# SeanNaren/deepspeech.pytorch

Hardware: AMD Instinct MI355X
Metric: audio-seconds/sec (train step) (higher is better)
Workload: dtype bf16

## Files before the change

deepspeech/pytorch_amd/_lib.py:

```python
import ctypes as C
import os

HERE = os.path.dirname(os.path.abspath(__file__))
LIB_PATH = os.path.join(HERE, "libds2hip.so")

F32, BF16 = 0, 1
CELL_GRU, CELL_LSTM, CELL_RNN_TANH = 0, 1, 2

_vp, _i, _l, _f, _ll = C.c_void_p, C.c_int, C.c_long, C.c_float, C.c_longlong

SIGNATURES = {
    "ds2_version": (_i, []),
    "ds2_error_string": (C.c_char_p, [_i]),
    "ds2_gemm_nt": (_i, [_i, _vp, _vp, _vp, _vp, _i, _i, _i, _l, _l, _l, _i, _i, _l, _l, _l, _l, _i, _vp]),
    "ds2_gemm_nt_coresident": (_i, [_i, _vp, _vp, _vp, _vp, _i, _i, _i, _l, _l, _l, _i, _i, _l, _l, _l, _l, _i, _vp]),
    "ds2_gemm_nt_rows2": (_i, [_i, _vp, _vp, _i, _vp, _vp, _i, _i, _i, _l, _l, _l, _i, _i, _i, _vp]),
    "ds2_gemm8_nt": (_i, [_vp, _vp, _vp, _vp, _i, _i, _i, _l, _l, _l, _i, _vp]),
    "ds2_gemm8_tn_grouped": (_i, [_i, _vp, _vp, _vp, _vp, _vp, _vp, _vp, _vp, _vp, _vp, _vp, _i, _vp]),
    "ds2_gemm8_nt_rows": (_i, [_vp, _vp, _vp, _vp, _i, _i, _i, _l, _l, _l, _i, _vp, _i, _vp]),
    "ds2_gemm8_tn_grouped_rows": (_i, [_i, _vp, _vp, _vp, _vp, _vp, _vp, _vp, _vp, _vp, _vp, _vp, _i, _vp, _i, _vp]),
    "ds2_gemm8_wgrad_dx_rows": (_i, [_i, _vp, _vp, _vp, _vp, _vp, _vp, _vp, _vp, _vp, _vp, _vp, _i, _vp, _vp, _vp, _i, _i, _i, _l, _l, _l, _vp, _i, _vp]),
    "ds2_zero_pad_rows": (_i, [_i, _vp, _l, _i, _vp, _i, _i, _vp]),
    "ds2_gemm8_wgrad_dx": (_i, [_i, _vp, _vp, _vp, _vp, _vp, _vp, _vp, _vp, _vp, _vp, _vp, _i, _vp, _vp, _vp, _i, _i, _i, _l, _l, _l, _vp]),
    "ds2_norm_partials": (_i, [_l]),
    "ds2_bn_fwd": (_i, [_i, _i, _i, _vp, _vp, _l, _i, _l, _l, _i, _i, _i, _vp, _vp, _vp, _vp, _vp, _vp, _f, _f, _vp, _vp,
                        _vp, _vp, _vp, _vp]),
    "ds2_bn_bwd": (_i, [_i, _i, _vp, _vp, _vp, _l, _i, _l, _l, _l, _i, _i, _i, _vp, _vp, _vp, _vp, _vp, _vp, _vp, _vp, _vp]),
    "ds2_colsum": (_i, [_i, _vp, _l, _i, _l, _vp, _f, _vp, _vp]),
    "ds2_conv_rows": (_i, [_i, _vp, _vp]),
    "ds2_conv1_fwd": (_i, [_i, _vp, _vp, _vp, _vp, _vp, _i, _i, _i, _i, _vp]),
    "ds2_conv1_wgrad_ws_floats": (_l, [_i, _i, _i]),
    "ds2_conv1_wgrad": (_i, [_i, _vp, _vp, _vp, _i, _i, _i, _i, _vp, _vp]),
    "ds2_conv2_fwd_ws_bytes": (_l, [_i, _i, _i, _i]),
    "ds2_conv2_fwd": (_i, [_i, _vp, _vp, _vp, _vp, _vp, _i, _i, _i, _vp, _vp]),
    "ds2_conv2_dgrad": (_i, [_i, _vp, _vp, _vp, _vp, _i, _i, _i, _vp]),
    "ds2_conv2_wgrad_ws_floats": (_l, [_i, _i]),
    "ds2_conv2_wgrad": (_i, [_i, _vp, _vp, _vp, _i, _i, _i, _vp, _vp]),
    "ds2_rnn_gates": (_i, [_i]),
    "ds2_rnn_saved_planes": (_i, [_i]),
    "ds2_rnn_state_bytes": (_l, [_i, _i, _i]),
    "ds2_rnn_fwd": (_i, [_i, _i, _i, _i, _i, _i, _vp, _vp, _vp, _vp, _vp, _vp, _vp, _l, _vp, _vp, _vp, _vp, _vp]),
    "ds2_rnn_bwd": (_i, [_i, _i, _i, _i, _i, _i, _vp, _vp, _vp, _vp, _l, _vp, _vp, _vp, _vp, _vp, _vp, _vp, _vp, _vp]),
    "ds2_rnn_persist_plan": (_i, [_i, _i, _i, _i, _i, _i, C.c_uint, C.POINTER(_l)]),
    "ds2_rnn_persist_supported": (_i, [_i, _i, _i, _i, _i, C.c_uint]),
    "ds2_rnn_persist_shape_covered": (_i, [_i, _i, _i, _i, _i]),
    "ds2_rnn_persist_kind": (_i, [_i, _i, _i, _i, _i, C.c_uint]),
    "ds2_rnn_persist_ws_bytes": (_l, [_i, _i, _i, _i, _i, C.c_uint]),
    "ds2_rnn_persist_fwd": (_i, [_i, _i, _i, _i, _i, _i, _vp, _vp, _vp, _vp, _vp, _vp, _vp, _l, _vp, _vp, _vp, _vp, _vp, _vp, _vp]),
    "ds2_rnn_persist_bwd": (_i, [_i, _i, _i, _i, _i, _i, _vp, _vp, _vp, _vp, _l, _vp, _vp, _vp, _vp, _i, _vp, _vp, _vp, _vp]),
    "ds2_add2": (_i, [_i, _vp, _vp, _vp, _l, _vp]),
    "ds2_sum_slices": (_i, [_vp, _vp, _l, _i, _vp]),
    "ds2_transpose": (_i, [_i, _vp, _vp, _l, _i, _l, _l, _vp]),
    "ds2_split3_bf16": (_i, [_vp, _l, _l, _i, _i, _i, _vp, _l, _vp]),
    "ds2_cast_transpose_bf16": (_i, [_vp, _l, _i, _i, _i, _i, _i, _vp, _l, _vp, _l, _vp]),
    "ds2_small_weight_layouts": (_i, [_i, _vp, _vp, _vp, _i, _i, _vp, _vp, _vp, _vp, _vp, _vp, _vp]),
    "ds2_scale_by": (_i, [_vp, _vp, _l, _vp]),
    "ds2_copy_words": (_i, [_vp, _vp, _l, _vp]),
    "ds2_lookahead_fwd": (_i, [_i, _vp, _vp, _vp, _vp, _i, _i, _i, _i, _vp]),
    "ds2_lookahead_ws_floats": (_l, [_i, _i, _i, _i]),
    "ds2_lookahead_bwd": (_i, [_i, _vp, _vp, _vp, _vp, _vp, _vp, _i, _i, _i, _i, _vp, _vp]),
    "ds2_rnn_bias_grads": (_i, [_i, _i, _i, _i, _vp, _vp, _vp, _vp]),
# ... 69 lines not shown
```

deepspeech/pytorch_amd/csrc/ds2_norm.hip:

```cpp
#include "ds2_common.h"

namespace {

constexpr int NORM_RY = 8;
constexpr int NORM_CX = 32;

struct RowMap {
  int F, Tp;
  __device__ __forceinline__ void nt(long row, int& n, int& t) const {
    t = (int)(row % Tp);
    n = (int)(row / ((long)F * Tp));
  }
};

__device__ __forceinline__ float bn_affine(float x, float sc, float sh) { return __builtin_fmaf(x, sc, sh); }
__device__ __forceinline__ bool hardtanh_open(float y) { return y > 0.f && y < 20.f; }
__device__ __forceinline__ float bn_dx(float g, float xh, float sc, float k1, float k2) { return sc * __builtin_fmaf(-xh, k2, g - k1); }

struct RedMap {
  int cpb, rpx, chunk, rsub;
  bool ok;
  __device__ __forceinline__ RedMap(int chunks) {
    cpb = chunks < NORM_CX ? chunks : NORM_CX;
    rpx = NORM_CX / cpb;
// ... 28 lines not shown
                                                                float* __restrict__ psum, float* __restrict__ psq) {
  constexpr int V = Vec16<T>::N;
  __shared__ float red[NORM_RY][NORM_CX * V + 1];
  const RedMap m(C / V);
  float s[V], q[V];
#pragma unroll
  for (int i = 0; i < V; ++i) s[i] = q[i] = 0.f;
  if (m.ok) {
    for (long r = m.first_row(); r < R; r += m.row_step()) {
      float v[V];
      Vec16<T>::load(X + r * ld + (long)m.chunk * V, v);
#pragma unroll
      for (int i = 0; i < V; ++i) {
        s[i] += v[i];
        if (SQ) q[i] += v[i] * v[i];
      }
    }
  }
  float o[V];
  red_block<V>(red, m, s, o);
  if (threadIdx.y == 0 && m.rsub == 0 && m.ok) {
#pragma unroll
    for (int i = 0; i < V; ++i) psum[(long)blockIdx.y * C + (long)m.chunk * V + i] = o[i];
  }
  if (SQ) {
    red_block<V>(red, m, q, o);
    if (threadIdx.y == 0 && m.rsub == 0 && m.ok) {
#pragma unroll
      for (int i = 0; i < V; ++i) psq[(long)blockIdx.y * C + (long)m.chunk * V + i] = o[i];
    }
  }
}

constexpr int FIN_COLS = 32, FIN_SLICES = 8;
template <int NA>
__device__ __forceinline__ void finalize_sums(const float* const (&arr)[NA], int P, int C, int c, int py, double (&tot)[NA]) {
  __shared__ double sh[NA][FIN_SLICES][FIN_COLS];
  double acc[NA];
#pragma unroll
  for (int a = 0; a < NA; ++a) acc[a] = 0.0;
  if (c < C) {
#pragma unroll 8
    for (int p = py; p < P; p += FIN_SLICES) {
#pragma unroll
      for (int a = 0; a < NA; ++a) acc[a] += (double)arr[a][(long)p * C + c];
    }
  }
#pragma unroll
  for (int a = 0; a < NA; ++a) sh[a][py][threadIdx.x & (FIN_COLS - 1)] = acc[a];
  __syncthreads();
#pragma unroll
  for (int a = 0; a < NA; ++a) {
    double t = 0.0;
    if (py == 0) {
#pragma unroll
      for (int q = 0; q < FIN_SLICES; ++q) t += sh[a][q][threadIdx.x & (FIN_COLS - 1)];
    }
    tot[a] = t;
  }
}

__global__ void __launch_bounds__(256) k_colsum_finalize(const float* __restrict__ psum, int P, int C, float* __restrict__ out,
                                                          float scale) {
  const int c = blockIdx.x * FIN_COLS + (threadIdx.x & (FIN_COLS - 1)), py = threadIdx.x / FIN_COLS;
  const float* const arr[1] = {psum};
  double tot[1];
  finalize_sums<1>(arr, P, C, c, py, tot);
  if (py == 0 && c < C) out[c] = (float)(tot[0] * (double)scale);
}

__global__ void k_bn_finalize(const float* __restrict__ psum, const float* __restrict__ psq, int P, int C, double count,
                              const float* __restrict__ gamma, const float* __restrict__ beta, float eps,
                              float momentum, float* __restrict__ running_mean, float* __restrict__ running_var,
                              long long* __restrict__ num_batches_tracked, float* __restrict__ mean_out,
                              float* __restrict__ rstd_out, float* __restrict__ scale_out, float* __restrict__ shift_out) {
  const int c = blockIdx.x * FIN_COLS + (threadIdx.x & (FIN_COLS - 1)), py = threadIdx.x / FIN_COLS;
  if (blockIdx.x == 0 && threadIdx.x == 0 && num_batches_tracked) *num_batches_tracked += 1;
  const float* const arr[2] = {psum, psq};
  double tot[2];
  finalize_sums<2>(arr, P, C, c, py, tot);
  if (py != 0 || c >= C) return;
  const double s = tot[0], q = tot[1];
  double mean = s / count;
  double var = q / count - mean * mean;
  if (var < 0.0) var = 0.0;
  double rstd = 1.0 / sqrt(var + (double)eps);
  mean_out[c] = (float)mean;
  rstd_out[c] = (float)rstd;
  float sc = (float)((double)gamma[c] * rstd);
  scale_out[c] = sc;
  shift_out[c] = (float)((double)beta[c] - mean * (double)gamma[c] * rstd);
  if (running_mean) {
    double unb = count > 1.0 ? var * (count / (count - 1.0)) : var;
    running_mean[c] = (float)((1.0 - (double)momentum) * (double)running_mean[c] + (double)momentum * mean);
    running_var[c] = (float)((1.0 - (double)momentum) * (double)running_var[c] + (double)momentum * unb);
  }
}

__global__ void k_bn_eval_coeffs(int C, const float* __restrict__ gamma, const float* __restrict__ beta,
                                 const float* __restrict__ running_mean, const float* __restrict__ running_var, float eps,
                                 float* __restrict__ scale_out, float* __restrict__ shift_out) {
  int c = blockIdx.x * blockDim.x + threadIdx.x;
  if (c >= C) return;
  double rstd = 1.0 / sqrt((double)running_var[c] + (double)eps);
  scale_out[c] = (float)((double)gamma[c] * rstd);
  shift_out[c] = (float)((double)beta[c] - (double)running_mean[c] * (double)gamma[c] * rstd);
}

template <typename T, bool CONV, bool SEQ_OUT, bool CENTRED = false>
__global__ void __launch_bounds__(256) k_bn_apply(const T* __restrict__ X, T* __restrict__ Y, long R, int C, long ldx,
                                                   long ldy, const float* __restrict__ scale,
                                                   const float* __restrict__ shift, const float* __restrict__ mean,
                                                   const float* __restrict__ beta, RowMap rm,
                                                   const int* __restrict__ lens, int N) {
  constexpr int V = Vec16<T>::N;
  const int chunks = C / V;
  const long total = R * chunks;
  for (long e = (long)blockIdx.x * blockDim.x + threadIdx.x; e < total; e += (long)gridDim.x * blockDim.x) {
    long r = e / chunks;
    int c0 = (int)(e % chunks) * V;
    float v[V];
    bool live = true;
    int n = 0, t = 0;
    if (CONV) {
      rm.nt(r, n, t);
// ... 225 lines not shown
  else
    hipLaunchKernelGGL((k_colstats<T, false>), grd, blk, 0, st, (const T*)X, R, C, ld, psum, psq);
  *P_out = grd.y;
  DS2_CHECK_LAUNCH();
  return 0;
}

inline int apply_grid(long total) {
  long g = (total + 255) / 256;
  if (g > 256 * 8) g = 256 * 8;
  if (g < 1) g = 1;
  return (int)g;
}

}

extern "C" {

int ds2_norm_partials(long R) { return norm_grid_y(R); }

int ds2_colsum(int dtype, const void* X, long R, int C, long ld, float* out, float scale, float* ws, ds2_stream_t st_) {
  hipStream_t st = (hipStream_t)st_;
  int P = 0, rc;
  if (dtype == DS2_F32)
    rc = colstats_impl<float>(X, R, C, ld, ws, nullptr, &P, st);
  else
    rc = colstats_impl<bf16_t>(X, R, C, ld, ws, nullptr, &P, st);
  if (rc) return rc;
  hipLaunchKernelGGL(k_colsum_finalize, dim3(ds2_cdiv(C, FIN_COLS)), dim3(256), 0, st, ws, P, C, out, scale);
  DS2_CHECK_LAUNCH();
  return 0;
}

int ds2_bn_fwd(int dtype, int mode, int training, const void* X, void* Y, long R, int C, long ldx, long ldy, int F, int Tp,
               int N, const int* lens, const float* gamma, const float* beta, float* running_mean, float* running_var,
               long long* num_batches_tracked, float eps, float momentum, float* save_mean, float* save_rstd,
               float* save_scale, float* save_shift, float* ws, ds2_stream_t st_) {
  hipStream_t st = (hipStream_t)st_;
  DS2_REQUIRE(dtype == DS2_F32 || dtype == DS2_BF16, DS2_ERR_DTYPE);
  DS2_REQUIRE(mode >= 0 && mode <= 2, DS2_ERR_ARG);
  DS2_REQUIRE(mode == 0 || R < (1L << 31), DS2_ERR_ARG);
  int rc, P = 0;
  if (training) {
    float* psum = ws;
    float* psq = ws + (long)norm_grid_y(R) * C;
    rc = dtype == DS2_F32 ? colstats_impl<float>(X, R, C, ldx, psum, psq, &P, st)
                          : colstats_impl<bf16_t>(X, R, C, ldx, psum, psq, &P, st);
    if (rc) return rc;
    hipLaunchKernelGGL(k_bn_finalize, dim3(ds2_cdiv(C, FIN_COLS)), dim3(256), 0, st, psum, psq, P, C, (double)R, gamma, beta,
                       eps, momentum, running_mean, running_var, num_batches_tracked, save_mean, save_rstd, save_scale,
                       save_shift);
  } else {
    hipLaunchKernelGGL(k_bn_eval_coeffs, dim3(ds2_cdiv(C, 128)), dim3(128), 0, st, C, gamma, beta, running_mean,
                       running_var, eps, save_scale, save_shift);
  }
  DS2_CHECK_LAUNCH();
  RowMap rm{F, Tp};
  const int V = dtype == DS2_F32 ? 4 : 8;
  DS2_REQUIRE(C % V == 0 && ldx % V == 0 && ldy % V == 0, DS2_ERR_ALIGN);
  dim3 g(apply_grid(R * (C / V))), b(256);
#define LAUNCH_APPLY(TT)                                                                                              \
  if (mode == 0 && training && R == 1)                                                                                \
    hipLaunchKernelGGL((k_bn_apply<TT, false, false, true>), g, b, 0, st, (const TT*)X, (TT*)Y, R, C, ldx, ldy,        \
                       save_scale, save_shift, save_mean, beta, rm, lens, N);                                         \
  else if (mode == 0)                                                                                                 \
    hipLaunchKernelGGL((k_bn_apply<TT, false, false>), g, b, 0, st, (const TT*)X, (TT*)Y, R, C, ldx, ldy, save_scale,  \
                       save_shift, save_mean, beta, rm, lens, N);                                                     \
  else if (mode == 1)                                                                                                 \
    hipLaunchKernelGGL((k_bn_apply<TT, true, false>), g, b, 0, st, (const TT*)X, (TT*)Y, R, C, ldx, ldy, save_scale,   \
                       save_shift, save_mean, beta, rm, lens, N);                                                     \
  else                                                                                                                \
    hipLaunchKernelGGL((k_bn_apply<TT, true, true>), g, b, 0, st, (const TT*)X, (TT*)Y, R, C, ldx, ldy, save_scale,    \
                       save_shift, save_mean, beta, rm, lens, N);
  if (dtype == DS2_F32) {
    LAUNCH_APPLY(float)
  } else {
    LAUNCH_APPLY(bf16_t)
  }
#undef LAUNCH_APPLY
  DS2_CHECK_LAUNCH();
  return 0;
}

int ds2_bn_bwd(int dtype, int mode, const void* G, const void* X, void* DX, long R, int C, long ldg, long ldx, long lddx,
               int F, int Tp, int N, const int* lens, const float* save_mean, const float* save_rstd,
               const float* save_scale, const float* save_shift, float* dgamma, float* dbeta, float* ws, ds2_stream_t st_) {
  hipStream_t st = (hipStream_t)st_;
  DS2_REQUIRE(dtype == DS2_F32 || dtype == DS2_BF16, DS2_ERR_DTYPE);
  DS2_REQUIRE(mode >= 0 && mode <= 2, DS2_ERR_ARG);
  DS2_REQUIRE(mode == 0 || R < (1L << 31), DS2_ERR_ARG);
  const int V = dtype == DS2_F32 ? 4 : 8;
  DS2_REQUIRE(C % V == 0 && ldx % V == 0 && ldg % V == 0 && lddx % V == 0, DS2_ERR_ALIGN);
  RowMap rm{F, Tp};
  const int P = norm_grid_y(R, ds2_cdiv(C / V, NORM_CX));
  float* ps = ws;
  float* pq = ws + (long)P * C;
  float* c1 = pq + (long)P * C;
  float* c2 = c1 + C;
  dim3 blk(NORM_CX, NORM_RY), grd(ds2_cdiv(C / V, NORM_CX), P);
#define LAUNCH_RED(TT, CV, SI)                                                                                          \
  hipLaunchKernelGGL((k_bn_bwd_reduce<TT, CV, SI>), grd, blk, 0, st, (const TT*)G, (const TT*)X, R, C, ldg, ldx,          \
                     save_scale, save_shift, save_mean, save_rstd, rm, lens, N, ps, pq)
  const int acb = ds2_cdiv(C / V, NORM_CX), arpx = NORM_CX / (C / V < NORM_CX ? C / V : NORM_CX);
  long agy = ds2_cdiv(R, (long)NORM_RY * arpx * 2);
  if (agy > 2048 / acb) agy = 2048 / acb;
  if (agy < 1) agy = 1;
  const dim3 agrd(acb, (unsigned)agy);
#ifdef DS2_BN_APPLY_GRIDSTRIDE
#define LAUNCH_APP(TT, CV, SI)                                                                                          \
  hipLaunchKernelGGL((k_bn_bwd_apply<TT, CV, SI>), dim3(apply_grid(R*(C / V))), dim3(256), 0, st, (const TT*)G,           \
                     (const TT*)X, (TT*)DX, R, C, ldg, ldx, lddx, save_scale, save_shift, save_mean, save_rstd, c1, c2, \
                     rm, lens, N)
// ... 30 lines not shown
```

deepspeech/pytorch_amd/model.py:

```python
import math
from typing import List

import numpy as np
import torch
import torch.nn as nn

from . import ops
from ._lib import Ds2HipError

try:
    import pytorch_lightning as pl
    _Base = pl.LightningModule
except Exception:
    pl = None

    class _Base(nn.Module):

        def save_hyperparameters(self, *a, **k):
            import inspect
            frame = inspect.currentframe().f_back
            try:
                names = [n for n in inspect.signature(type(self).__init__).parameters if n != "self"]
                self._hparams = {n: frame.f_locals[n] for n in names if n in frame.f_locals}
            finally:
# ... 159 lines not shown
    def clear(self):
        self._store.clear()


def _wgrad_splitk(M, N, K):
    tiles = ((M + 127) // 128) * ((N + 127) // 128)
    if tiles >= 128:
        return 1
    return max(1, min(8, 768 // max(tiles, 1), K // (64 * 32)))


def _pad_gate_rows(w, G, H, Hp):
    if Hp == H:
        return w
    out = w.new_zeros((G, Hp) + tuple(w.shape[1:]))
    out[:, :H] = w.reshape((G, H) + tuple(w.shape[1:]))
    return out.reshape((G * Hp,) + tuple(w.shape[1:]))


def _pad_cols(w, Cp):
    if w.shape[-1] == Cp:
        return w
    out = w.new_zeros(tuple(w.shape[:-1]) + (Cp,))
    out[..., :w.shape[-1]] = w
    return out


def _unpad_gate_rows(g, G, H, Hp):
    if Hp == H:
        return g
    return g.reshape((G, Hp) + tuple(g.shape[1:]))[:, :H].reshape((G * H,) + tuple(g.shape[1:])).contiguous()


def _bn_seq_fwd(bn, w, b, X, Xh, R, Ct, Cp, training):
    if Ct == Cp:
        return ops.bn_fwd(X, 0, training, w.detach(), b.detach(), bn.running_mean, bn.running_var, bn.num_batches_tracked, R, Ct,
                          X.stride(0), Xh, Xh.stride(0), eps=bn.eps, momentum=bn.momentum)
    g, be = w.new_ones(Cp), w.new_zeros(Cp)
    rm, rv = w.new_zeros(Cp), w.new_ones(Cp)
    g[:Ct], be[:Ct], rm[:Ct], rv[:Ct] = w.detach(), b.detach(), bn.running_mean, bn.running_var
    sv = ops.bn_fwd(X, 0, training, g, be, rm, rv, bn.num_batches_tracked, R, Cp, X.stride(0), Xh, Xh.stride(0), eps=bn.eps,
                    momentum=bn.momentum)
    if training:
        bn.running_mean.copy_(rm[:Ct])
        bn.running_var.copy_(rv[:Ct])
    return sv


def _bn_seq_bwd(G, X, DX, sv, R, Ct, Cp):
    dg, db = ops.bn_bwd(G, X, DX, 0, sv, R, Cp, G.stride(0), X.stride(0), DX.stride(0))
    return (dg, db) if Ct == Cp else (dg[:Ct].contiguous(), db[:Ct].contiguous())


def _perm_cols_to_internal(w):
    g, rin = w.shape
    out = w.new_zeros((g, _round64(rin)))
    out[:, :rin] = w.reshape(g, 32, rin // 32).permute(0, 2, 1).reshape(g, rin)
    return out


def _perm_cols_to_reference(w, rin=RNN_INPUT):
    g = w.shape[0]
    return w[:, :rin].reshape(g, rin // 32, 32).permute(0, 2, 1).reshape(g, rin)


class _ConvStackFn(torch.autograd.Function):

# ... 73 lines not shown
    R = Tp * N
    layer = mod.rnns[li]
    kind, Ht, D = layer.kind, layer.hidden_size, layer.num_directions
    H = mod._Hp
    G = ops.GATES[kind]
    first = li == 0
    I = mod._rnn_ld if first else H
    has_bn = layer.batch_norm is not None
    bn_w, bn_b = (lparams[0], lparams[1]) if has_bn else (None, None)
    wts = lparams[2 if has_bn else 0:]
    wih = [wts[4 * d + 0] for d in range(D)]
    whh = [wts[4 * d + 1] for d in range(D)]
    bih = [wts[4 * d + 2] for d in range(D)]
    bhh = [wts[4 * d + 3] for d in range(D)]

    def build_ih():
        w = torch.cat([_pad_gate_rows(p.detach(), G, Ht, H) for p in wih], 0)
        w = _perm_cols_to_internal(w) if first else _pad_cols(w, H)
        out = ops.empty_padded(w.shape[0], w.shape[1], dtype, w.device)
        out.copy_(w)
        return out
    Wih = c.get(("wih", li, dtype), wih, build_ih)
    Whh = c.get(("whh", li, dtype), whh, lambda: torch.stack(
        [_pad_gate_rows(_pad_cols(p.detach(), H), G, Ht, H) for p in whh], 0).to(dtype).contiguous())
    if H == Ht:
        Bih, Bhh = mod._bias_views(li)
    else:
        Bih = c.get(("bih", li), bih, lambda: torch.cat([_pad_gate_rows(p.detach(), G, Ht, H) for p in bih], 0))
        Bhh = c.get(("bhh", li), bhh, lambda: torch.stack([_pad_gate_rows(p.detach(), G, Ht, H) for p in bhh], 0))
    sv, Xh = None, X
    if has_bn:
        bn = layer.batch_norm.module
        Xh = ops.empty_padded(R, I, X.dtype, X.device)
        sv = _bn_seq_fwd(bn, bn_w, bn_b, X, Xh, R, layer.input_size, I, training)
    if ops.split3_ok(dtype, R, D * G * H, I):
        Wih3 = c.get(("wih3", li), wih, lambda: ops.split3(Wih, 1))
        GI = ops.gemm_nt(ops.split3(Xh, 0), Wih3, bias=Bih, out_dtype=torch.float32, rows=rows)
    else:
        GI = ops.gemm_nt(Xh, Wih, bias=Bih, rows=rows)
    if H != Ht:
        h0 = _pad_cols(h0, H) if h0 is not None else None
        c0 = _pad_cols(c0, H) if c0 is not None else None
    hext, Sv, hn, cn = ops.rnn_fwd(kind, GI, Whh, Bhh, lens_dev, D, N, H, Tp, h0=h0, c0=c0)
    if H != Ht:
        hn = hn[..., :Ht].contiguous()
        cn = cn[..., :Ht].contiguous() if cn is not None else None
    del GI
    if D == 2:
        out = ops.add2(hext[0, 1:Tp + 1].reshape(R, H), hext[1, 1:Tp + 1].reshape(R, H))
    else:
        out = hext[0, 1:Tp + 1].reshape(R, H)
    return out, hn, cn, [X, Xh if has_bn else None, hext, Sv], (kind, H, D, G, I, has_bn, sv, Ht, layer.input_size)


def _rnn_layer_backward(mod, li, meta, saved, lparams, dout, lens_dev, N, Tp, dtype, main, side, rows=None, state=None):
    kind, H, D, G, I, has_bn, sv, Ht, It = meta
    if state is not None:
        h0, c0, want = state
        h0p = _pad_cols(h0, H) if (h0 is not None and H != Ht) else h0
        c0p = _pad_cols(c0, H) if (c0 is not None and H != Ht) else c0
        state = (h0p, c0p, bool(want))
    dX, grads, rg = _rnn_layer_backward_impl(mod, li, meta, saved, lparams, dout, lens_dev, N, Tp, dtype, main, side, rows, state)
    if state is None:
        return dX, grads, None
    main.wait_stream(side)
    GH, po = G * H, (2 if has_bn else 0)
    if h0p is not None:
        n4 = (N + 3) // 4 * 4
        ar = torch.arange(N, device=lens_dev.device)
        for d in range(D):
            t_first = torch.zeros_like(ar) if d == 0 else (lens_dev.long().clamp(1, Tp) - 1)
            src = rg.dGH[d].reshape(Tp * N, GH) if (kind == "gru" and rg.dGH is not None) else rg.dGI[:, d * GH:(d + 1) * GH]
            g_first = src.index_select(0, t_first * N + ar).float()
            A = torch.zeros((GH, n4), dtype=torch.float32, device=g_first.device)
            A[:, :N] = g_first.t()
            B = torch.zeros((H, n4), dtype=torch.float32, device=g_first.device)
            B[:, :N] = h0p[d].t()
            corr = ops.gemm_nt(A, B, out_dtype=torch.float32)
            grads[po + 4 * d + 1] = grads[po + 4 * d + 1] + _unpad_gate_rows(corr, G, Ht, H)[:, :Ht]
    dstate = None
    if want:
        dstate = (rg.dh0[..., :Ht].contiguous(), rg.dc0[..., :Ht].contiguous() if rg.dc0 is not None else None)
# ... 512 lines not shown
            nn.BatchNorm2d(32),
            nn.Hardtanh(0, 20, inplace=True)
        ))
        rnn_input_size = int(math.floor((self.spect_cfg.sample_rate * self.spect_cfg.window_size) / 2) + 1)
        rnn_input_size = int(math.floor(rnn_input_size + 2 * 20 - 41) / 2 + 1)
        rnn_input_size = int(math.floor(rnn_input_size + 2 * 10 - 21) / 2 + 1)
        rnn_input_size *= 32
        self._F0 = int(math.floor((self.spect_cfg.sample_rate * self.spect_cfg.window_size) / 2) + 1)
        self._F1, self._F2 = ops.conv_rows(self._F0)
        self._rnn_in, self._rnn_ld = 32 * self._F2, _round64(32 * self._F2)
        if rnn_input_size != self._rnn_in or self._F2 < 1:
            raise ValueError("unsupported spectrogram geometry: %d frequency bins" % self._F0)
        self.rnns = nn.Sequential(
            BatchRNN(rnn_input_size, H, kind, bidirectional=self.bidirectional, batch_norm=False),
            *(BatchRNN(H, H, kind, bidirectional=self.bidirectional) for _ in range(L - 1))
        )
        self.lookahead = nn.Sequential(
            Lookahead(H, context=model_cfg.lookahead_context),
            nn.Hardtanh(0, 20, inplace=True)
        ) if not self.bidirectional else None
        fully_connected = nn.Sequential(nn.BatchNorm1d(H), nn.Linear(H, num_classes, bias=False))
        self.fc = nn.Sequential(SequenceWise(fully_connected))
        self.blank_index = self.labels.index('_')
        from .decoder import GreedyDecoder
        self.inference_softmax = InferenceBatchSoftmax()
        self.criterion = CTCLossHip(blank=self.blank_index)
        self.evaluation_decoder = GreedyDecoder(self.labels, blank_index=self.blank_index)
        self.wer, self.cer = _reference_metrics(self.evaluation_decoder)
        self._cache = _WeightCache()
        self._flat_bias = {}
        self._side_streams = {}
        self._prep_done = None
        self._frame_rows = None
        self._weights_dirty = False
        self._kind = kind

    def _prep_rnn_weights(self, dtype, need_backward):
        c = self._cache
        if self._Hp != self.rnns[0].hidden_size:
            return
        for li, layer in enumerate(self.rnns):
            p, D, first = layer.rnn, layer.num_directions, li == 0
            sufs = [""] + (["_reverse"] if D == 2 else [])
            wih = [getattr(p, "weight_ih_l0" + s_) for s_ in sufs]
            whh = [getattr(p, "weight_hh_l0" + s_) for s_ in sufs]
            bih = [getattr(p, "bias_ih_l0" + s_) for s_ in sufs]
            bhh = [getattr(p, "bias_hh_l0" + s_) for s_ in sufs]

            if dtype == torch.bfloat16:
                keys = [("wih", li, dtype), ("whh", li, dtype)]
                if need_backward:
                    keys += [("wihT", li, dtype), ("whhT", li, dtype)]
                if not all(c.valid(k, wih if k[0].startswith("wih") else whh) for k in keys):
                    GH, H = whh[0].shape
                    I = wih[0].shape[1]
                    Io = self._rnn_ld if first else I
                    perm = (32, self._F2) if first else None
                    dev = wih[0].device
                    Wih = ops.empty_padded(D * GH, Io, dtype, dev)
                    Whh = torch.empty((D, GH, H), dtype=dtype, device=dev)
                    WihT = torch.empty((Io, D * GH), dtype=dtype, device=dev) if need_backward else None
                    WhhT = torch.empty((D, H, GH), dtype=dtype, device=dev) if need_backward else None
                    with torch.no_grad():
                        for d in range(D):
                            ops.cast_transpose_bf16(wih[d].detach(), Wih[d * GH:], Wih.stride(0),
                                                    WihT[:, d * GH:] if need_backward else None, D * GH, perm=perm, cout=Io)
# ... 225 lines not shown
```

deepspeech/pytorch_amd/ops.py:

```python
import ctypes as C

import numpy as np
import torch

from . import _lib
from ._lib import F32, BF16, call, query

CELLS = {"gru": _lib.CELL_GRU, "lstm": _lib.CELL_LSTM, "rnn": _lib.CELL_RNN_TANH}
GATES = {"gru": 3, "lstm": 4, "rnn": 1}
SAVED_PLANES = {"gru": 4, "lstm": 5, "rnn": 0}


def dt(t):
    d = t if isinstance(t, torch.dtype) else t.dtype
    if d == torch.float32:
        return F32
    if d == torch.bfloat16:
        return BF16
    raise TypeError("ds2hip supports float32 and bfloat16 activations, got %s" % d)


def vecw(dtype):
    return 4 if dtype == torch.float32 else 8

# ... 260 lines not shown
    return out


def cast_transpose_bf16(src, dst=None, ldd=0, dstT=None, lddT=0, perm=None, cout=None):
    R, Cc = src.shape
    pc, pf = perm if perm is not None else (0, 0)
    call("ds2_cast_transpose_bf16", PF(src), src.stride(0), R, Cc, pc, pf, Cc if cout is None else cout,
         P(dst) if dst is not None else None, ldd, P(dstT) if dstT is not None else None, lddT, S())


def small_weight_layouts(w1, w2, wfc, dtype):
    dev, Cc, H = w1.device, wfc.shape[0], wfc.shape[1]
    w1k = torch.empty((451, 32), dtype=torch.float32, device=dev)
    w2t = torch.empty((21, 11, 32, 32), dtype=dtype, device=dev)
    w2d0 = torch.empty((11, 11, 32, 32), dtype=dtype, device=dev)
    w2d1 = torch.empty((10, 11, 32, 32), dtype=dtype, device=dev)
    wp = torch.empty((32, H), dtype=dtype, device=dev)
    wpT = torch.empty((H, 32), dtype=dtype, device=dev)
    call("ds2_small_weight_layouts", dt(dtype), PF(w1), PF(w2), PF(wfc), Cc, H, P(w1k), P(w2t), P(w2d0), P(w2d1), P(wp), P(wpT), S())
    return w1k, w2t, [w2d0, w2d1], wp, wpT


def scale_by_(x, s):
    call("ds2_scale_by", P(x), PF(s.reshape(1)), x.numel(), S())
    return x


def add2(a, b):
    out = torch.empty_like(a)
    call("ds2_add2", dt(a), P(a), P(b), P(out), a.numel(), S())
    return out


class BnSaved:
    __slots__ = ("mean", "rstd", "scale", "shift")

    def __init__(self, Cc, device):
        buf = torch.empty((4, Cc), dtype=torch.float32, device=device)
        self.mean, self.rstd, self.scale, self.shift = buf[0], buf[1], buf[2], buf[3]


def bn_fwd(X, mode, training, gamma, beta, rmean, rvar, nbt, R, Cc, ldx, Y, ldy, F=0, Tp=0, N=0, lens=None, eps=1e-5,
           momentum=0.1):
    sv = BnSaved(Cc, X.device)
    ws = torch.empty(2 * query("ds2_norm_partials", R) * Cc, dtype=torch.float32, device=X.device)
    call("ds2_bn_fwd", dt(X), mode, 1 if training else 0, P(X), P(Y), R, Cc, ldx, ldy, F, Tp, N, P(lens), PF(gamma), PF(beta),
         PF(rmean), PF(rvar), P(nbt) if training else C.c_void_p(0), float(eps), float(momentum), P(sv.mean), P(sv.rstd),
         P(sv.scale), P(sv.shift), P(ws), S())
    return sv


def bn_bwd(G, X, DX, mode, sv, R, Cc, ldg, ldx, lddx, F=0, Tp=0, N=0, lens=None):
    dgamma = torch.empty(Cc, dtype=torch.float32, device=X.device)
    dbeta = torch.empty(Cc, dtype=torch.float32, device=X.device)
    ws = torch.empty((2 * query("ds2_norm_partials", R) + 2) * Cc, dtype=torch.float32, device=X.device)
    call("ds2_bn_bwd", dt(X), mode, P(G), P(X), P(DX), R, Cc, ldg, ldx, lddx, F, Tp, N, P(lens), P(sv.mean), P(sv.rstd),
         P(sv.scale), P(sv.shift), P(dgamma), P(dbeta), P(ws), S())
    return dgamma, dbeta


def conv_rows(F0):
    F1 = (F0 + 2 * 20 - 41) // 2 + 1
    return F1, (F1 + 2 * 10 - 21) // 2 + 1


def conv1_fwd(x, w1k, b1, lens, Tp, dtype):
    N, _, F0, T = x.shape
    y1 = torch.empty((N, conv_rows(F0)[0], Tp, 32), dtype=dtype, device=x.device)
    call("ds2_conv1_fwd", dt(dtype), PF(x), PF(w1k), PF(b1), P(lens), P(y1), N, F0, T, Tp, S())
    return y1


def conv1_wgrad(x, dy1, Tp):
    N, _, F0, T = x.shape
    dw = torch.empty((451, 32), dtype=torch.float32, device=x.device)
    ws = torch.empty(query("ds2_conv1_wgrad_ws_floats", N, F0, Tp), dtype=torch.float32, device=x.device)
    call("ds2_conv1_wgrad", dt(dy1), P(x), P(dy1), P(dw), N, F0, T, Tp, P(ws), S())
    return dw


def conv2_fwd(a1, w2t, b2, lens, F0=161):
# ... 220 lines not shown
def use_persistent(kind, dtype, D, N, H):
    if not PERSIST_ENABLED:
        return False
    ok = bool(query("ds2_rnn_persist_supported", dt(dtype), CELLS[kind], D, N, H, int(_OPTS["variant"])))
    if ok:
        return True
    import os
    import warnings
    covered = bool(query("ds2_rnn_persist_shape_covered", dt(dtype), CELLS[kind], D, N, H))
    if covered:
        dev = torch.cuda.current_device()
        cus = torch.cuda.get_device_properties(dev).multi_processor_count
        if os.environ.get("DS2_ALLOW_LAUNCH_PER_STEP", "0") in ("", "0"):
            raise _lib.Ds2HipError("ds2hip: device %d exposes %d compute units (< 256): the persistent recurrent kernels need one "
                                   "workgroup per CU, all co-resident.  Set DS2_ALLOW_LAUNCH_PER_STEP=1 to run the launch-per-time-step "
                                   "kernels instead (several times slower)." % (dev, cus))
        if dev not in _WARNED_CUS:
            _WARNED_CUS.add(dev)
            warnings.warn("ds2hip: device %d exposes %d compute units (< 256): the persistent recurrent kernels are disabled, the "
                          "recurrent sweeps use one launch per time step" % (dev, cus))
    elif H >= PERSIST_CLIFF_MIN_H:
        key = (kind, str(dtype), D, N, H)
        if key not in _WARNED_SHAPES:
            _WARNED_SHAPES.add(key)
            widths = [w for w in range(16, 2049, 16) if query("ds2_rnn_persist_shape_covered", dt(dtype), CELLS[kind], D, N, w)]
            warnings.warn("ds2hip: no persistent recurrent kernel is instantiated for %s %s hidden=%d, %d direction(s), batch %d: the "
                          "sweeps run one launch per time step (5-8x slower per step).  For this cell, type, direction count and batch "
                          "persistent kernels exist with hidden in {%s}; the model class zero-pads other hidden sizes up to the nearest "
                          "instantiated width when that is at most 1.5x as wide (DS2_PAD_HIDDEN)."
                          % (str(dtype).replace("torch.", ""), kind, H, D, N, ", ".join(map(str, widths))))
    return False


def rnn_fwd(kind, GI, Whh, bhh, lens, D, N, H, Tp, h0=None, c0=None, save=True):
    dev, dtype = GI.device, GI.dtype
    hext = torch.empty((D, Tp + 2, N, H), dtype=dtype, device=dev)
    persistent = use_persistent(kind, dtype, D, N, H)
    if not persistent:
        hext[:, 0].zero_()
        hext[:, Tp + 1].zero_()
    ns = SAVED_PLANES[kind]
    Sv = torch.empty((D, Tp, N, max(ns, 1) * H) if ns else (1,), dtype=dtype, device=dev)
    hn = torch.empty((D, N, H), dtype=torch.float32, device=dev)
    cn = torch.empty((D, N, H), dtype=torch.float32, device=dev) if kind == "lstm" else None
    if persistent:
        ws = torch.empty(query("ds2_rnn_persist_ws_bytes", dt(dtype), CELLS[kind], D, N, H, int(_OPTS["variant"])), dtype=torch.uint8, device=dev)
        global LAST_PERSIST_WS
        LAST_PERSIST_WS = ws
        po = _persist_opts()
        with _sweep_timer("rnn_fwd_persistent", Tp):
            call("ds2_rnn_persist_fwd", dt(dtype), CELLS[kind], D, N, H, Tp, P(lens), P(GI), P(Whh), PF(bhh), PF(h0), PF(c0),
                 P(hext[:, 1]), (Tp + 2) * N * H, P(Sv), P(hn), P(cn), P(ws), P(_persist_err(dev)), C.byref(po), S())
        return hext, Sv, hn, cn
    state = torch.empty(query("ds2_rnn_state_bytes", D, N, H), dtype=torch.uint8, device=dev)
    with _sweep_timer("rnn_fwd", Tp):
        call("ds2_rnn_fwd", dt(dtype), CELLS[kind], D, N, H, Tp, P(lens), P(GI), P(Whh), PF(bhh), PF(h0), PF(c0),
             P(hext[:, 1]), (Tp + 2) * N * H, P(Sv), P(hn), P(cn), P(state), S())
    return hext, Sv, hn, cn


class RnnGrads:
    __slots__ = ("dGI", "dGH", "dQ", "bacc", "dh0", "dc0")

    def __init__(self, dGI, dGH=None, dQ=None, bacc=None):
        self.dGI, self.dGH, self.dQ, self.bacc = dGI, dGH, dQ, bacc
        self.dh0 = self.dc0 = None

    def tensors(self):
        return [t for t in (self.dGI, self.dGH, self.dQ, self.bacc) if t is not None]
# ... 340 lines not shown
```

include/ds2hip.h:

```cpp
#ifndef DS2HIP_H
#define DS2HIP_H

#include <stdint.h>

#ifdef __cplusplus
extern "C" {
#endif

typedef void* ds2_stream_t;

enum { DS2_F32 = 0, DS2_BF16 = 1 };
enum { DS2_CELL_GRU = 0, DS2_CELL_LSTM = 1, DS2_CELL_RNN_TANH = 2 };
enum {
  DS2_OK = 0,
  DS2_ERR_DTYPE = 1001,
  DS2_ERR_ARG = 1002,
  DS2_ERR_ALIGN = 1003
};

int ds2_version(void);
const char* ds2_error_string(int code);

int ds2_gemm_nt(int dtype, const void* A, const void* B, void* C, const float* bias, int M, int N, int K, long lda, long ldb,
                long ldc, int out_f32, int batch, long strideA, long strideB, long strideC, long strideBias, int splitk,
// ... 1 lines not shown

int ds2_gemm_nt_rows2(int dtype, const void* A, const void* A2, int m_split, const void* B, void* C, int M, int N, int K, long lda,
                      long ldb, long ldc, int out_f32, int splitk, int coresident, ds2_stream_t stream);
int ds2_gemm_nt_coresident(int dtype, const void* A, const void* B, void* C, const float* bias, int M, int N, int K, long lda,
                           long ldb, long ldc, int out_f32, int batch, long strideA, long strideB, long strideC, long strideBias,
                           int splitk, ds2_stream_t stream);

int ds2_gemm8_nt(const void* A, const void* B, void* C, const float* bias, int M, int N, int K, long lda, long ldb, long ldc, int out_f32,
                 ds2_stream_t stream);
int ds2_gemm8_tn_grouped(int n_problems, const void* const* At, const void* const* At2, const int* m_split, const void* const* Bt, void* const* C,
                         const int* M, const int* N, const long* lda, const long* lda2, const long* ldb, const long* ldc, int K, ds2_stream_t stream);

int ds2_gemm8_wgrad_dx(int n_tn, const void* const* At, const void* const* At2, const int* m_split, const void* const* Bt, void* const* C,
                       const int* M, const int* N, const long* lda, const long* lda2, const long* ldb, const long* ldc, int K_tn,
                       const void* A_nt, const void* B_nt, void* C_nt, int M_nt, int N_nt, int K_nt, long lda_nt, long ldb_nt, long ldc_nt,
                       ds2_stream_t stream);

int ds2_gemm8_nt_rows(const void* A, const void* B, void* C, const float* bias, int n_phys, int N, int K, long lda, long ldb, long ldc,
                      int out_f32, const int* rows, int n_rows, ds2_stream_t stream);
int ds2_gemm8_tn_grouped_rows(int n_problems, const void* const* At, const void* const* At2, const int* m_split, const void* const* Bt,
                              void* const* C, const int* M, const int* N, const long* lda, const long* lda2, const long* ldb, const long* ldc,
                              int n_phys, const int* rows, int n_rows, ds2_stream_t stream);
int ds2_gemm8_wgrad_dx_rows(int n_tn, const void* const* At, const void* const* At2, const int* m_split, const void* const* Bt, void* const* C,
                            const int* M, const int* N, const long* lda, const long* lda2, const long* ldb, const long* ldc, int K_tn,
                            const void* A_nt, const void* B_nt, void* C_nt, int M_nt, int N_nt, int K_nt, long lda_nt, long ldb_nt, long ldc_nt,
                            const int* rows, int n_rows, ds2_stream_t stream);
int ds2_zero_pad_rows(int dtype, void* X, long ld, int cols, const int* lens, int Tp, int N, ds2_stream_t stream);

int ds2_norm_partials(long R);
int ds2_bn_fwd(int dtype, int mode, int training, const void* X, void* Y, long R, int C, long ldx, long ldy, int F, int Tp,
               int N, const int* lens, const float* gamma, const float* beta, float* running_mean, float* running_var,
               long long* num_batches_tracked, float eps, float momentum, float* save_mean, float* save_rstd,
               float* save_scale, float* save_shift, float* ws, ds2_stream_t stream);
int ds2_bn_bwd(int dtype, int mode, const void* G, const void* X, void* DX, long R, int C, long ldg, long ldx, long lddx,
               int F, int Tp, int N, const int* lens, const float* save_mean, const float* save_rstd,
               const float* save_scale, const float* save_shift, float* dgamma, float* dbeta, float* ws,
               ds2_stream_t stream);
int ds2_colsum(int dtype, const void* X, long R, int C, long ld, float* out, float scale, float* ws, ds2_stream_t stream);

int ds2_conv_rows(int F0, int* F1, int* F2);
int ds2_conv1_fwd(int dtype, const float* x, const float* w1k, const float* b1, const int* lens, void* y1, int N, int F0, int T,
                  int Tp, ds2_stream_t stream);
long ds2_conv1_wgrad_ws_floats(int N, int F0, int Tp);
int ds2_conv1_wgrad(int dtype, const float* x, const void* dy1, float* dw1k, int N, int F0, int T, int Tp, float* ws,
                    ds2_stream_t stream);
long ds2_conv2_fwd_ws_bytes(int dtype, int N, int F0, int Tp);
int ds2_conv2_fwd(int dtype, const void* a1, const void* w2t, const float* b2, const int* lens, void* y2, int N, int F0, int Tp,
                  void* ws, ds2_stream_t stream);
int ds2_conv2_dgrad(int dtype, const void* dy2, const void* w2d_even, const void* w2d_odd, void* da1, int N, int F0, int Tp,
                    ds2_stream_t stream);
long ds2_conv2_wgrad_ws_floats(int N, int Tp);
int ds2_conv2_wgrad(int dtype, const void* dy2, const void* a1, float* dw2t, int N, int F0, int Tp, float* ws, ds2_stream_t stream);

int ds2_rnn_gates(int cell);
int ds2_rnn_saved_planes(int cell);
long ds2_rnn_state_bytes(int D, int N, int H);
int ds2_rnn_fwd(int dtype, int cell, int D, int N, int H, int Tp, const int* lens, const void* GI, const void* Whh,
                const float* bhh, const float* h0, const float* c0, void* Hseq, long hseq_dstride, void* S, float* hn, float* cn,
                void* state, ds2_stream_t stream);
int ds2_rnn_bwd(int dtype, int cell, int D, int N, int H, int Tp, const int* lens, const void* dOut, const void* WhhT,
                const void* Hseq, long hseq_dstride, const void* S, void* dGI, void* dGH, const float* h0, const float* c0,
                float* dh0, float* dc0, void* state, ds2_stream_t stream);

typedef struct ds2_persist_opts {
  unsigned variant;
  unsigned spin_limit;
// ... 91 lines not shown
```

Before: 21460.

## Fuse bidirectional sum with next layer's batch-norm column statistics

When a bidirectional RNN layer feeds a batch-normalized layer in training, the direction sum now also computes per-column partial sums and squared sums in the same pass. The next layer's BN forward reuses these partials and skips its own column-statistics read over the activation. A new seq-BN entry point also handles padded channels (Ct < C) directly, avoiding a separate slice path. This saves one full read of each inter-layer activation plus a launch, at the cost of extra bookkeeping to validate the cached stats by pointer and version, and stats are computed on rounded bf16 values.

```diff
diff --git a/deepspeech/pytorch_amd/_lib.py b/deepspeech/pytorch_amd/_lib.py
--- a/deepspeech/pytorch_amd/_lib.py
+++ b/deepspeech/pytorch_amd/_lib.py
@@ -27,6 +27,8 @@
                         _vp, _vp, _vp, _vp]),
     "ds2_bn_bwd": (_i, [_i, _i, _vp, _vp, _vp, _l, _i, _l, _l, _l, _i, _i, _i, _vp, _vp, _vp, _vp, _vp, _vp, _vp, _vp, _vp]),
     "ds2_colsum": (_i, [_i, _vp, _l, _i, _l, _vp, _f, _vp, _vp]),
+    "ds2_bn_seq_train_fwd": (_i, [_i, _vp, _vp, _l, _i, _i, _l, _l, _vp, _vp, _vp, _vp, _vp, _f, _f, _vp, _vp, _vp, _vp, _vp, _i, _vp]),
+    "ds2_add2_colstats": (_i, [_i, _vp, _vp, _vp, _l, _i, _l, _l, _l, _vp, _vp]),
     "ds2_conv_rows": (_i, [_i, _vp, _vp]),
     "ds2_conv1_fwd": (_i, [_i, _vp, _vp, _vp, _vp, _vp, _i, _i, _i, _i, _vp]),
     "ds2_conv1_wgrad_ws_floats": (_l, [_i, _i, _i]),
diff --git a/deepspeech/pytorch_amd/csrc/ds2_norm.hip b/deepspeech/pytorch_amd/csrc/ds2_norm.hip
--- a/deepspeech/pytorch_amd/csrc/ds2_norm.hip
+++ b/deepspeech/pytorch_amd/csrc/ds2_norm.hip
@@ -84,6 +84,79 @@
   }
 }
 
+template <typename T>
+struct StoreRounded;
+template <>
+struct StoreRounded<float> {
+  static __device__ __forceinline__ void run(float* p, float (&v)[4]) { Vec16<float>::store(p, v); }
+};
+template <>
+struct StoreRounded<bf16_t> {
+  static __device__ __forceinline__ void run(bf16_t* p, float (&v)[8]) {
+    uint32_t w[4];
+#pragma unroll
+    for (int i = 0; i < 4; ++i) w[i] = cvt_pk_bf16(v[2 * i], v[2 * i + 1]);
+    *reinterpret_cast<uint4*>(p) = make_uint4(w[0], w[1], w[2], w[3]);
+#pragma unroll
+    for (int i = 0; i < 4; ++i) {
+      v[2 * i] = __uint_as_float(w[i] << 16);
+      v[2 * i + 1] = __uint_as_float(w[i] & 0xffff0000u);
+    }
+  }
+};
+
+template <typename T>
+__global__ void __launch_bounds__(NORM_RY* NORM_CX) k_add2_colstats(const T* __restrict__ A, const T* __restrict__ B, T* __restrict__ O,
+                                                                     long R, int C, long lda, long ldb, long ldo,
+                                                                     float* __restrict__ psum, float* __restrict__ psq) {
+  constexpr int V = Vec16<T>::N;
+  __shared__ float red[NORM_RY][NORM_CX * V + 1];
+  const RedMap m(C / V);
+  float s[V], q[V];
+#pragma unroll
+  for (int i = 0; i < V; ++i) s[i] = q[i] = 0.f;
+  if (m.ok) {
+    const long c0 = (long)m.chunk * V, step = m.row_step();
+    auto finish = [&](long r, float (&a)[V], const float (&b)[V]) {
+#pragma unroll
+      for (int i = 0; i < V; ++i) a[i] += b[i];
+      StoreRounded<T>::run(O + r * ldo + c0, a);
+#pragma unroll
+      for (int i = 0; i < V; ++i) {
+        s[i] += a[i];
+        q[i] += a[i] * a[i];
+      }
+    };
+    long r = m.first_row();
+    for (; r + step < R; r += 2 * step) {
+      float a0[V], b0[V], a1[V], b1[V];
+      Vec16<T>::load(A + r * lda + c0, a0);
+      Vec16<T>::load(B + r * ldb + c0, b0);
+      Vec16<T>::load(A + (r + step) * lda + c0, a1);
+      Vec16<T>::load(B + (r + step) * ldb + c0, b1);
+      finish(r, a0, b0);
+      finish(r + step, a1, b1);
+    }
+    if (r < R) {
+      float a0[V], b0[V];
+      Vec16<T>::load(A + r * lda + c0, a0);
+      Vec16<T>::load(B + r * ldb + c0, b0);
+      finish(r, a0, b0);
+    }
+  }
+  float o[V];
+  red_block<V>(red, m, s, o);
+  if (threadIdx.y == 0 && m.rsub == 0 && m.ok) {
+#pragma unroll
+    for (int i = 0; i < V; ++i) psum[(long)blockIdx.y * C + (long)m.chunk * V + i] = o[i];
+  }
+  red_block<V>(red, m, q, o);
+  if (threadIdx.y == 0 && m.rsub == 0 && m.ok) {
+#pragma unroll
+    for (int i = 0; i < V; ++i) psq[(long)blockIdx.y * C + (long)m.chunk * V + i] = o[i];
+  }
+}
+
 constexpr int FIN_COLS = 32, FIN_SLICES = 8;
 template <int NA>
 __device__ __forceinline__ void finalize_sums(const float* const (&arr)[NA], int P, int C, int c, int py, double (&tot)[NA]) {
@@ -121,7 +194,7 @@
   if (py == 0 && c < C) out[c] = (float)(tot[0] * (double)scale);
 }
 
-__global__ void k_bn_finalize(const float* __restrict__ psum, const float* __restrict__ psq, int P, int C, double count,
+__global__ void k_bn_finalize(const float* __restrict__ psum, const float* __restrict__ psq, int P, int C, int Ct, double count,
                               const float* __restrict__ gamma, const float* __restrict__ beta, float eps,
                               float momentum, float* __restrict__ running_mean, float* __restrict__ running_var,
                               long long* __restrict__ num_batches_tracked, float* __restrict__ mean_out,
@@ -139,10 +212,11 @@
   double rstd = 1.0 / sqrt(var + (double)eps);
   mean_out[c] = (float)mean;
   rstd_out[c] = (float)rstd;
-  float sc = (float)((double)gamma[c] * rstd);
+  const float ga = c < Ct ? gamma[c] : 1.f, be = c < Ct ? beta[c] : 0.f;
+  float sc = (float)((double)ga * rstd);
   scale_out[c] = sc;
-  shift_out[c] = (float)((double)beta[c] - mean * (double)gamma[c] * rstd);
-  if (running_mean) {
+  shift_out[c] = (float)((double)be - mean * (double)ga * rstd);
+  if (running_mean && c < Ct) {
     double unb = count > 1.0 ? var * (count / (count - 1.0)) : var;
     running_mean[c] = (float)((1.0 - (double)momentum) * (double)running_mean[c] + (double)momentum * mean);
     running_var[c] = (float)((1.0 - (double)momentum) * (double)running_var[c] + (double)momentum * unb);
@@ -434,22 +508,32 @@
   return 0;
 }
 
-int ds2_bn_fwd(int dtype, int mode, int training, const void* X, void* Y, long R, int C, long ldx, long ldy, int F, int Tp,
-               int N, const int* lens, const float* gamma, const float* beta, float* running_mean, float* running_var,
-               long long* num_batches_tracked, float eps, float momentum, float* save_mean, float* save_rstd,
-               float* save_scale, float* save_shift, float* ws, ds2_stream_t st_) {
+}
+
+namespace {
+int bn_fwd_impl(int dtype, int mode, int training, const void* X, void* Y, long R, int C, int Ct, long ldx, long ldy, int F, int Tp,
+                int N, const int* lens, const float* gamma, const float* beta, float* running_mean, float* running_var,
+                long long* num_batches_tracked, float eps, float momentum, float* save_mean, float* save_rstd,
+                float* save_scale, float* save_shift, float* ws, bool have_stats, ds2_stream_t st_) {
   hipStream_t st = (hipStream_t)st_;
   DS2_REQUIRE(dtype == DS2_F32 || dtype == DS2_BF16, DS2_ERR_DTYPE);
   DS2_REQUIRE(mode >= 0 && mode <= 2, DS2_ERR_ARG);
   DS2_REQUIRE(mode == 0 || R < (1L << 31), DS2_ERR_ARG);
+  DS2_REQUIRE(Ct >= 0 && Ct <= C && R > 0, DS2_ERR_ARG);
   int rc, P = 0;
   if (training) {
     float* psum = ws;
     float* psq = ws + (long)norm_grid_y(R) * C;
-    rc = dtype == DS2_F32 ? colstats_impl<float>(X, R, C, ldx, psum, psq, &P, st)
-                          : colstats_impl<bf16_t>(X, R, C, ldx, psum, psq, &P, st);
-    if (rc) return rc;
-    hipLaunchKernelGGL(k_bn_finalize, dim3(ds2_cdiv(C, FIN_COLS)), dim3(256), 0, st, psum, psq, P, C, (double)R, gamma, beta,
+    if (have_stats) {
+      const int V = dtype == DS2_F32 ? 4 : 8;
+      DS2_REQUIRE(C % V == 0, DS2_ERR_ALIGN);
+      P = norm_grid_y(R, ds2_cdiv(C / V, NORM_CX));
+    } else {
+      rc = dtype == DS2_F32 ? colstats_impl<float>(X, R, C, ldx, psum, psq, &P, st)
+                            : colstats_impl<bf16_t>(X, R, C, ldx, psum, psq, &P, st);
+      if (rc) return rc;
+    }
+    hipLaunchKernelGGL(k_bn_finalize, dim3(ds2_cdiv(C, FIN_COLS)), dim3(256), 0, st, psum, psq, P, C, Ct, (double)R, gamma, beta,
                        eps, momentum, running_mean, running_var, num_batches_tracked, save_mean, save_rstd, save_scale,
                        save_shift);
   } else {
@@ -480,6 +564,47 @@
     LAUNCH_APPLY(bf16_t)
   }
 #undef LAUNCH_APPLY
+  DS2_CHECK_LAUNCH();
+  return 0;
+}
+}
+
+extern "C" {
+
+int ds2_bn_fwd(int dtype, int mode, int training, const void* X, void* Y, long R, int C, long ldx, long ldy, int F, int Tp,
+               int N, const int* lens, const float* gamma, const float* beta, float* running_mean, float* running_var,
+               long long* num_batches_tracked, float eps, float momentum, float* save_mean, float* save_rstd,
+               float* save_scale, float* save_shift, float* ws, ds2_stream_t st_) {
+  return bn_fwd_impl(dtype, mode, training, X, Y, R, C, C, ldx, ldy, F, Tp, N, lens, gamma, beta, running_mean, running_var,
+                     num_batches_tracked, eps, momentum, save_mean, save_rstd, save_scale, save_shift, ws, false, st_);
+}
+
+int ds2_bn_seq_train_fwd(int dtype, const void* X, void* Y, long R, int C, int Ct, long ldx, long ldy, const float* gamma,
+                         const float* beta, float* running_mean, float* running_var, long long* num_batches_tracked, float eps,
+                         float momentum, float* save_mean, float* save_rstd, float* save_scale, float* save_shift, float* ws,
+                         int have_stats, ds2_stream_t st_) {
+  return bn_fwd_impl(dtype, 0, 1, X, Y, R, C, Ct, ldx, ldy, 0, 0, 0, nullptr, gamma, beta, running_mean, running_var,
+                     num_batches_tracked, eps, momentum, save_mean, save_rstd, save_scale, save_shift, ws, have_stats != 0, st_);
+}
+
+int ds2_add2_colstats(int dtype, const void* a, const void* b, void* out, long R, int C, long lda, long ldb, long ldo, float* ws,
+                      ds2_stream_t st_) {
+  hipStream_t st = (hipStream_t)st_;
+  DS2_REQUIRE(dtype == DS2_F32 || dtype == DS2_BF16, DS2_ERR_DTYPE);
+  DS2_REQUIRE(a && b && out && ws && R > 0 && C > 0 && lda >= C && ldb >= C && ldo >= C, DS2_ERR_ARG);
+  const int V = dtype == DS2_F32 ? 4 : 8;
+  DS2_REQUIRE(C % V == 0 && lda % V == 0 && ldb % V == 0 && ldo % V == 0, DS2_ERR_ALIGN);
+  DS2_REQUIRE(((((uintptr_t)a) | ((uintptr_t)b) | ((uintptr_t)out)) & 15) == 0, DS2_ERR_ALIGN);
+  float* psum = ws;
+  float* psq = ws + (long)norm_grid_y(R) * C;
+  dim3 blk(NORM_CX, NORM_RY);
+  dim3 grd(ds2_cdiv(C / V, NORM_CX), norm_grid_y(R, ds2_cdiv(C / V, NORM_CX)));
+  if (dtype == DS2_F32)
+    hipLaunchKernelGGL(k_add2_colstats<float>, grd, blk, 0, st, (const float*)a, (const float*)b, (float*)out, R, C, lda, ldb, ldo,
+                       psum, psq);
+  else
+    hipLaunchKernelGGL(k_add2_colstats<bf16_t>, grd, blk, 0, st, (const bf16_t*)a, (const bf16_t*)b, (bf16_t*)out, R, C, lda, ldb,
+                       ldo, psum, psq);
   DS2_CHECK_LAUNCH();
   return 0;
 }
diff --git a/deepspeech/pytorch_amd/model.py b/deepspeech/pytorch_amd/model.py
--- a/deepspeech/pytorch_amd/model.py
+++ b/deepspeech/pytorch_amd/model.py
@@ -215,7 +215,10 @@
     return g.reshape((G, Hp) + tuple(g.shape[1:]))[:, :H].reshape((G * H,) + tuple(g.shape[1:])).contiguous()
 
 
-def _bn_seq_fwd(bn, w, b, X, Xh, R, Ct, Cp, training):
+def _bn_seq_fwd(bn, w, b, X, Xh, R, Ct, Cp, training, stats=None):
+    if training and w.is_contiguous() and b.is_contiguous():
+        return ops.bn_seq_train_fwd(X, w.detach(), b.detach(), bn.running_mean, bn.running_var, bn.num_batches_tracked, R, Cp, Ct,
+                                    X.stride(0), Xh, Xh.stride(0), eps=bn.eps, momentum=bn.momentum, stats=stats)
     if Ct == Cp:
         return ops.bn_fwd(X, 0, training, w.detach(), b.detach(), bn.running_mean, bn.running_var, bn.num_batches_tracked, R, Ct,
                           X.stride(0), Xh, Xh.stride(0), eps=bn.eps, momentum=bn.momentum)
@@ -355,7 +358,13 @@
     if has_bn:
         bn = layer.batch_norm.module
         Xh = ops.empty_padded(R, I, X.dtype, X.device)
-        sv = _bn_seq_fwd(bn, bn_w, bn_b, X, Xh, R, layer.input_size, I, training)
+        ahead, mod._bn_stats_ahead = getattr(mod, "_bn_stats_ahead", None), None
+        stats = None
+        if ahead is not None and training and ahead[0].data_ptr() == X.data_ptr() and ahead[0].shape == X.shape and \
+                ahead[0].dtype == X.dtype and X.is_contiguous() and ahead[2] == X._version:
+            stats = ahead[1]
+        del ahead
+        sv = _bn_seq_fwd(bn, bn_w, bn_b, X, Xh, R, layer.input_size, I, training, stats=stats)
     if ops.split3_ok(dtype, R, D * G * H, I):
         Wih3 = c.get(("wih3", li), wih, lambda: ops.split3(Wih, 1))
         GI = ops.gemm_nt(ops.split3(Xh, 0), Wih3, bias=Bih, out_dtype=torch.float32, rows=rows)
@@ -370,7 +379,12 @@
         cn = cn[..., :Ht].contiguous() if cn is not None else None
     del GI
     if D == 2:
-        out = ops.add2(hext[0, 1:Tp + 1].reshape(R, H), hext[1, 1:Tp + 1].reshape(R, H))
+        above = mod.rnns[li + 1] if li + 1 < len(mod.rnns) else None
+        if training and above is not None and above.batch_norm is not None:
+            out, stats = ops.add2_colstats(hext[0, 1:Tp + 1].reshape(R, H), hext[1, 1:Tp + 1].reshape(R, H))
+            mod._bn_stats_ahead = (out, stats, out._version)
+        else:
+            out = ops.add2(hext[0, 1:Tp + 1].reshape(R, H), hext[1, 1:Tp + 1].reshape(R, H))
     else:
         out = hext[0, 1:Tp + 1].reshape(R, H)
     return out, hn, cn, [X, Xh if has_bn else None, hext, Sv], (kind, H, D, G, I, has_bn, sv, Ht, layer.input_size)
@@ -949,6 +963,7 @@
         self._side_streams = {}
         self._prep_done = None
         self._frame_rows = None
+        self._bn_stats_ahead = None
         self._weights_dirty = False
         self._kind = kind
 
diff --git a/deepspeech/pytorch_amd/ops.py b/deepspeech/pytorch_amd/ops.py
--- a/deepspeech/pytorch_amd/ops.py
+++ b/deepspeech/pytorch_amd/ops.py
@@ -316,6 +316,15 @@
     return out
 
 
+def add2_colstats(a, b):
+    R, Cc = a.shape
+    assert b.shape == a.shape and a.stride(1) == 1 and b.stride(1) == 1 and a.dtype == b.dtype
+    out = torch.empty((R, Cc), dtype=a.dtype, device=a.device)
+    ws = torch.empty(2 * query("ds2_norm_partials", R) * Cc, dtype=torch.float32, device=a.device)
+    call("ds2_add2_colstats", dt(a), P(a), P(b), P(out), R, Cc, a.stride(0), b.stride(0), Cc, P(ws), S())
+    return out, ws
+
+
 class BnSaved:
     __slots__ = ("mean", "rstd", "scale", "shift")
 
@@ -331,6 +340,16 @@
     call("ds2_bn_fwd", dt(X), mode, 1 if training else 0, P(X), P(Y), R, Cc, ldx, ldy, F, Tp, N, P(lens), PF(gamma), PF(beta),
          PF(rmean), PF(rvar), P(nbt) if training else C.c_void_p(0), float(eps), float(momentum), P(sv.mean), P(sv.rstd),
          P(sv.scale), P(sv.shift), P(ws), S())
+    return sv
+
+
+def bn_seq_train_fwd(X, gamma, beta, rmean, rvar, nbt, R, Cc, Ct, ldx, Y, ldy, eps=1e-5, momentum=0.1, stats=None):
+    sv = BnSaved(Cc, X.device)
+    ws = stats if stats is not None else torch.empty(2 * query("ds2_norm_partials", R) * Cc, dtype=torch.float32, device=X.device)
+    assert ws.numel() == 2 * query("ds2_norm_partials", R) * Cc and gamma.numel() == Ct and beta.numel() == Ct
+    assert (rmean is None) == (rvar is None) and (rmean is None or (rmean.numel() == Ct and rvar.numel() == Ct))
+    call("ds2_bn_seq_train_fwd", dt(X), P(X), P(Y), R, Cc, Ct, ldx, ldy, PF(gamma), PF(beta), PF(rmean), PF(rvar), P(nbt), float(eps),
+         float(momentum), P(sv.mean), P(sv.rstd), P(sv.scale), P(sv.shift), P(ws), 1 if stats is not None else 0, S())
     return sv
 
 
@@ -617,9 +636,11 @@
     return False
 
 
-def rnn_fwd(kind, GI, Whh, bhh, lens, D, N, H, Tp, h0=None, c0=None, save=True):
+def rnn_fwd(kind, GI, Whh, bhh, lens, D, N, H, Tp, h0=None, c0=None, save=True, hext=None):
     dev, dtype = GI.device, GI.dtype
-    hext = torch.empty((D, Tp + 2, N, H), dtype=dtype, device=dev)
+    if hext is None:
+        hext = torch.empty((D, Tp + 2, N, H), dtype=dtype, device=dev)
+    assert hext.shape == (D, Tp + 2, N, H) and hext.dtype == dtype and hext.is_contiguous()
     persistent = use_persistent(kind, dtype, D, N, H)
     if not persistent:
         hext[:, 0].zero_()
diff --git a/include/ds2hip.h b/include/ds2hip.h
--- a/include/ds2hip.h
+++ b/include/ds2hip.h
@@ -57,6 +57,12 @@
                int N, const int* lens, const float* gamma, const float* beta, float* running_mean, float* running_var,
                long long* num_batches_tracked, float eps, float momentum, float* save_mean, float* save_rstd,
                float* save_scale, float* save_shift, float* ws, ds2_stream_t stream);
+int ds2_bn_seq_train_fwd(int dtype, const void* X, void* Y, long R, int C, int Ct, long ldx, long ldy, const float* gamma,
+                         const float* beta, float* running_mean, float* running_var, long long* num_batches_tracked, float eps,
+                         float momentum, float* save_mean, float* save_rstd, float* save_scale, float* save_shift, float* ws,
+                         int have_stats, ds2_stream_t stream);
+int ds2_add2_colstats(int dtype, const void* a, const void* b, void* out, long R, int C, long lda, long ldb, long ldo, float* ws,
+                      ds2_stream_t stream);
 int ds2_bn_bwd(int dtype, int mode, const void* G, const void* X, void* DX, long R, int C, long ldg, long ldx, long lddx,
                int F, int Tp, int N, const int* lens, const float* save_mean, const float* save_rstd,
                const float* save_scale, const float* save_shift, float* dgamma, float* dbeta, float* ws,
```

Result: no change. 21420 (-0.2%).
